# Polarisjame/DeepFake

Hardware: AMD Instinct MI355X
Metric: train clips/sec (32x224x224 video + 16kHz audio) at 1/2/4/8 MI355X (higher is better)
Workload: dtype bf16; 1 GPU; C2: Swin-T video 32x224x224 (window 8x7x7) + SwinV2 mel 224 + wav2vec2-base 4s@16kHz + FusionModel, full train step; global_batch=8, per_gpu_batch=8, parallelism=dp1, hip_graph=True, captured_overlap=False, captured_bn_broadcast=False, branch_streams=3, regularisers=True

## Files before the change

deepfake_amd/_lib.py:

```python
import ctypes as C
import os

import torch

_HERE = os.path.dirname(os.path.abspath(__file__))
LIB_PATH = os.environ.get("DFK_LIB") or os.path.join(_HERE, "libdfk.so")

F32, BF16 = 0, 1


class Drop(C.Structure):
    _fields_ = [("rng", C.c_void_p), ("mode", C.c_int32), ("site", C.c_int32), ("p", C.c_float),
                ("group_rows", C.c_int32), ("shared", C.c_int32)]


class View(C.Structure):
    _fields_ = [("ptr", C.c_void_p), ("ld", C.c_int64), ("bs0", C.c_int64), ("bs1", C.c_int64),
                ("conv_cg", C.c_int32), ("conv_stride", C.c_int32), ("conv_pad", C.c_int32),
                ("conv_rows", C.c_int32)]


class GemmArgs(C.Structure):
    _fields_ = [("a", View), ("b", View), ("c", C.c_void_p), ("bias", C.c_void_p), ("residual", C.c_void_p),
                ("aux", C.c_void_p), ("ldc", C.c_int64), ("cbs0", C.c_int64), ("cbs1", C.c_int64),
                ("ldr", C.c_int64), ("rbs0", C.c_int64), ("rbs1", C.c_int64), ("ldaux", C.c_int64),
                ("bias_bs1", C.c_int64),
                ("M", C.c_int32), ("N", C.c_int32), ("K", C.c_int32), ("dtype", C.c_int32),
                ("a_kmajor", C.c_int32), ("b_kmajor", C.c_int32), ("c_f32", C.c_int32), ("nz0", C.c_int32),
                ("nz1", C.c_int32), ("splitk", C.c_int32), ("act", C.c_int32), ("atomic", C.c_int32),
                ("beta", C.c_float), ("ws", C.c_void_p), ("rowsum", C.c_void_p), ("drop", Drop),
                ("alpha", C.c_float), ("mx_q", C.c_void_p), ("mx_s", C.c_void_p), ("mx_ldq", C.c_int64),
                ("mx_lds", C.c_int64)]


class MxOperand(C.Structure):
    _fields_ = [("q", C.c_void_p), ("s", C.c_void_p), ("ld", C.c_int64), ("lds", C.c_int64)]


class WattnArgs(C.Structure):
    _fields_ = [("q", C.c_void_p), ("k", C.c_void_p), ("v", C.c_void_p), ("out", C.c_void_p),
                ("rpb", C.c_void_p), ("pad_q", C.c_void_p), ("pad_k", C.c_void_p), ("pad_v", C.c_void_p),
                ("lse", C.c_void_p), ("mask", C.c_void_p), ("mask_nw", C.c_int64),
                ("ld_qkv", C.c_int64), ("ld_out", C.c_int64),
                ("B", C.c_int32), ("D", C.c_int32), ("H", C.c_int32), ("W", C.c_int32),
                ("wd", C.c_int32), ("wh", C.c_int32), ("ww", C.c_int32),
                ("fd", C.c_int32), ("fh", C.c_int32), ("fw", C.c_int32),
                ("sd", C.c_int32), ("sh", C.c_int32), ("sw", C.c_int32),
                ("heads", C.c_int32), ("hd", C.c_int32), ("dtype", C.c_int32), ("scale", C.c_float),
                ("tab", C.c_void_p), ("drop", Drop), ("klen", C.c_void_p)]
# ... 26 lines not shown
                ("Ho", C.c_int32), ("Wo", C.c_int32)]


class Im2colArgs(C.Structure):
    _fields_ = [("sb", C.c_int64), ("sc", C.c_int64), ("st", C.c_int64), ("sh", C.c_int64), ("sw", C.c_int64),
                ("B", C.c_int32), ("cin", C.c_int32), ("T", C.c_int32), ("H", C.c_int32), ("W", C.c_int32),
                ("pd", C.c_int32), ("ph", C.c_int32), ("pw", C.c_int32),
                ("Do", C.c_int32), ("Ho", C.c_int32), ("Wo", C.c_int32)]


_VP, _I64, _I32, _F = C.c_void_p, C.c_int64, C.c_int32, C.c_float
SIGNATURES = {
    "dfk_gemm": [C.POINTER(GemmArgs), _VP],
    "dfk_gemm_workspace": [C.POINTER(GemmArgs)],
    "dfk_gemm_dw_group": [C.POINTER(GemmArgs), _I32, _VP],
    "dfk_colsum": [_VP, C.c_int, _I64, _I64, _I64, _VP, _VP],
    "dfk_gemm_mx": [C.POINTER(GemmArgs), C.POINTER(MxOperand), C.POINTER(MxOperand), _VP],
    "dfk_mx_quant": [_VP, C.c_int, _I64, _I64, _I64, C.c_int, _VP, _I64, _VP, _VP],
    "dfk_layernorm_fwd": [_VP, _VP, _VP, _VP, _VP, _VP, _I64, _I32, _F, C.c_int, _VP, C.POINTER(Drop), _VP],
    "dfk_layernorm_bwd": [_VP, _VP, _VP, _VP, _VP, _VP, _VP, _VP, _I64, _I32, C.c_int, C.c_int, _VP,
                          C.POINTER(Drop), _VP, _VP],
    "dfk_layernorm_bwd_workspace": [_I64, _I32],
    "dfk_wattn_fwd": [C.POINTER(WattnArgs), _VP],
    "dfk_wattn_bwd": [C.POINTER(WattnBwdArgs), _VP],
    "dfk_wattn_bwd_workspace": [C.POINTER(WattnArgs)],
    "dfk_wattn_fwd_policy": [C.c_int32, C.c_int64],
    "dfk_wattn_bwd_policy": [C.c_int32, C.c_int32],
    "dfk_wattn_table_workspace": [C.POINTER(WattnArgs)],
    "dfk_wattn_table": [C.POINTER(WattnArgs), _VP],
    "dfk_patch_im2col": [_VP, C.c_int, _VP, C.c_int, C.POINTER(Im2colArgs), _VP],
# ... 147 lines not shown
```

deepfake_amd/csrc/gemm.hip:

```cpp
#include <mutex>

#include "common.h"

namespace {

constexpr int NT = 256;

struct SplitK {
  float* slab;
  uint32_t* cnt;
};

template <typename T> struct GT;
template <> struct GT<bf16raw> { static constexpr int BK = 64, VEC = 8, PADR = 8, PADK = 16; };
template <> struct GT<float> { static constexpr int BK = 32, VEC = 4, PADR = 4, PADK = 4; };

template <typename T, bool KMAJ, int ROWS>
struct Tile {
  static constexpr int TBK = GT<T>::BK;
  static constexpr int STRIDE = KMAJ ? ROWS + GT<T>::PADK : TBK + GT<T>::PADR;
  static constexpr int ELEMS = KMAJ ? TBK * STRIDE : ROWS * STRIDE;
};

template <bool CONV>
// ... 176 lines not shown
      if (full) { float c8v[8]; ld8<T>(C, c8v); for (int e = 0; e < 8; ++e) v[e] += g.beta * c8v[e]; }
      else for (int e = 0; e < 8; ++e) if (e < ncol) v[e] += g.beta * ldf<T>(C + e);
    }
    if (full) st8<T>(C, v);
    else for (int e = 0; e < 8; ++e) if (e < ncol) stf<T>(C + e, v[e]);
  }
}

template <typename T, int WT, bool MXO = false>
__device__ __forceinline__ void tile_epilogue(const dfk_gemm_args& g, float* smem, const f32x4 (&acc)[WT / 16][WT / 16],
                                              int lane, int wave, int wm, int wn, int bm, int bn, int z, int split,
                                              int tile, int evec, SplitK sk);
__device__ __forceinline__ int mx_scale_byte(float am);
__device__ __forceinline__ uint2 mx_pack8(const float (&v)[8], int e);

template <typename T, int WT, bool AK, bool BKM, bool VECOK, bool CONV, bool RS = false>
__global__ __launch_bounds__(256) void gemm_kernel(const dfk_gemm_args g, int kchunk, int evec, SplitK sk) {
  constexpr int BM = 2 * WT, BN = 2 * WT, MI = WT / 16;
  constexpr int VA = tile_vecs<T, BM>(), VB = tile_vecs<T, BN>();
  using TA = Tile<T, AK, BM>;
  using TB = Tile<T, BKM, BN>;
  constexpr int TBK = GT<T>::BK;
  constexpr int BUF = TA::ELEMS + TB::ELEMS;
  constexpr int ES = WT + 4;
  constexpr int SMEM_T = 2 * BUF > (4 * WT * ES * 4) / (int)sizeof(T) ? 2 * BUF : (4 * WT * ES * 4) / (int)sizeof(T);
  __shared__ __attribute__((aligned(16))) T smem[SMEM_T];
  const int tid = threadIdx.x, lane = tid & 63, wave = tid >> 6;
  const int wm = wave >> 1, wn = wave & 1;
  int tn, tmi;
  {
    const int nwg = gridDim.x * gridDim.y, bid = blockIdx.y * gridDim.x + blockIdx.x;
    const int xcd = bid & 7, q = nwg >> 3, rr = nwg & 7;
    const int nid = (xcd < rr ? xcd * (q + 1) : rr * (q + 1) + (xcd - rr) * q) + (bid >> 3);
    tn = nid % gridDim.x;
    tmi = nid / gridDim.x;
  }
  const int bn = tn * BN, bm = tmi * BM;
  int z = blockIdx.z;
  const int split = z % g.splitk;
  z /= g.splitk;
  const int z0 = z / g.nz1, z1 = z % g.nz1;
  const T* A = reinterpret_cast<const T*>(g.a.ptr) + z0 * g.a.bs0 + z1 * g.a.bs1;
  const T* B = reinterpret_cast<const T*>(g.b.ptr) + z0 * g.b.bs0 + z1 * g.b.bs1;
  const int kbeg = split * kchunk;
  const int kend = min(g.K, kbeg + kchunk);

  f32x4 acc[MI][MI];
#pragma unroll
  for (int i = 0; i < MI; ++i)
#pragma unroll
    for (int j = 0; j < MI; ++j) acc[i][j] = f32x4{0.f, 0.f, 0.f, 0.f};
  const bool do_rs = RS && tn == 0 && wn == 0;
  f32x4 accr[MI];
// ... 73 lines not shown
      load_tile<T, BKM, BN, VECOK, CONV>(B, g.b, bn, g.N, kn, kend, tid, rb[nx]);
    }
  }

  if (RS && do_rs && (lane & 15) == 0) {
#pragma unroll
    for (int mi = 0; mi < MI; ++mi)
#pragma unroll
      for (int r = 0; r < 4; ++r) {
        const int row = bm + wm * WT + mi * 16 + (lane >> 4) * 4 + r;
        if (row < g.M) atomicAdd(g.rowsum + row, accr[mi][r]);
      }
  }
  __syncthreads();
  tile_epilogue<T, WT>(g, reinterpret_cast<float*>(smem), acc, lane, wave, wm, wn, bm, bn, z, split,
                       (z * (int)gridDim.y + tmi) * (int)gridDim.x + tn, evec, sk);
}

template <typename T, int WT, bool MXO>
__device__ __forceinline__ void tile_epilogue(const dfk_gemm_args& g, float* smem, const f32x4 (&acc)[WT / 16][WT / 16],
                                              int lane, int wave, int wm, int wn, int bm, int bn, int z, int split,
                                              int tile, int evec, SplitK sk) {
  constexpr int MI = WT / 16, ES = WT + 4;
  const int z0 = z / g.nz1, z1 = z % g.nz1;
  float* es = smem + wave * WT * ES;
#pragma unroll
  for (int mi = 0; mi < MI; ++mi)
#pragma unroll
    for (int ni = 0; ni < MI; ++ni)
#pragma unroll
      for (int r = 0; r < 4; ++r) es[(mi * 16 + (lane >> 4) * 4 + r) * ES + ni * 16 + (lane & 15)] = acc[mi][ni][r];
// ... 165 lines not shown
    const bf16raw* hi = img + (k + 4) * ROWS + ((c ^ kmaj_swz<ROWS>(k + 4)) << 3) + (p & 1) * 4;
    const short4v a = __builtin_amdgcn_ds_read_tr16_b64_v4i16((lds_short4*)(lo));
    const short4v b = __builtin_amdgcn_ds_read_tr16_b64_v4i16((lds_short4*)(hi));
    short8 u = {a[0], a[1], a[2], a[3], b[0], b[1], b[2], b[3]};
    return __builtin_bit_cast(bf16x8, u);
  }
}

__host__ __device__ __forceinline__ long view_extent(const dfk_view& v, long rows, long cols) {
  if (v.conv_cg > 0) return ((long)(v.conv_rows - 1) * v.ld + v.conv_cg) * 2;
  return ((rows - 1) * v.ld + cols) * 2;
}

constexpr int kRsPartialMin = 32;

template <int WT, int NWM, int NWN, bool AK, bool BKM, bool RS, bool CONV>
__device__ __forceinline__ void gemm_dma_body(const dfk_gemm_args& g, int kchunk, int evec, SplitK sk, const dim3 bid,
                                              const dim3 grid) {
  constexpr int NWV = NWM * NWN, BM = NWM * WT, BN = NWN * WT, MI = WT / 16, BK = 64, S = kStages;
  constexpr int STAGE = (BM + BN) * BK;
  constexpr int ES = WT + 4;
  constexpr int SMEM = S * STAGE * 2 > NWV * WT * ES * 4 ? S * STAGE * 2 : NWV * WT * ES * 4;
  __shared__ __attribute__((aligned(16))) float smem_f[SMEM / 4];
  bf16raw* smem = reinterpret_cast<bf16raw*>(smem_f);
  const int tid = threadIdx.x, lane = tid & 63;
  const int wave = __builtin_amdgcn_readfirstlane(tid >> 6);
  const int wm = wave / NWN, wn = wave % NWN;
  int tn, tmi, z;
  const int nwg = grid.x * grid.y;
  if (g.atomic && g.splitk % 8 == 0 && (int)grid.z == g.splitk && nwg > 1) {
    const int lin = bid.z * nwg + bid.y * grid.x + bid.x;
    const int j = lin >> 3, i = j % nwg;
    z = (j / nwg) * 8 + (lin & 7);
    tn = i % grid.x;
    tmi = i / grid.x;
  } else {
    const int b2 = bid.y * grid.x + bid.x;
    const int xcd = b2 & 7, q = nwg >> 3, rr = nwg & 7;
    const int nid = (xcd < rr ? xcd * (q + 1) : rr * (q + 1) + (xcd - rr) * q) + (b2 >> 3);
    tn = nid % grid.x;
    tmi = nid / grid.x;
    z = bid.z;
  }
  const int bn = tn * BN, bm = tmi * BM;
  const int split = z % g.splitk;
  z /= g.splitk;
  const int z0 = z / g.nz1, z1 = z % g.nz1;
  const bf16raw* A = reinterpret_cast<const bf16raw*>(g.a.ptr) + z0 * g.a.bs0 + z1 * g.a.bs1;
  const bf16raw* B = reinterpret_cast<const bf16raw*>(g.b.ptr) + z0 * g.b.bs0 + z1 * g.b.bs1;
  const __amdgpu_buffer_rsrc_t ra = __builtin_amdgcn_make_buffer_rsrc(
      const_cast<bf16raw*>(A), (short)0, (int)(AK ? view_extent(g.a, g.K, g.M) : view_extent(g.a, g.M, g.K)), 0x00020000);
  const __amdgpu_buffer_rsrc_t rb = __builtin_amdgcn_make_buffer_rsrc(
      const_cast<bf16raw*>(B), (short)0, (int)(BKM ? view_extent(g.b, g.K, g.N) : view_extent(g.b, g.N, g.K)), 0x00020000);
  const int kbeg = split * kchunk;
  const int kend = min(g.K, kbeg + kchunk);
  const int ntile = kend > kbeg ? (kend - kbeg + BK - 1) / BK : 0;

  auto issue = [&](int kt, bf16raw* st) {
    Dma<AK, BM, NWV, CONV>::issue(ra, g.a, bm, g.M, kt, kend, st, wave, lane);
// ... 69 lines not shown
            else atomicAdd(g.rowsum + row, accr[h][r]);
          }
        }
    }
  }
  asm volatile("s_waitcnt vmcnt(0) lgkmcnt(0)" ::: "memory");
  __syncthreads();
  tile_epilogue<bf16raw, WT>(g, smem_f, acc, lane, wave, wm, wn, bm, bn, z, split,
                             (z * (int)grid.y + tmi) * (int)grid.x + tn, evec, sk);
}

template <int WT, int NWM, int NWN, bool AK, bool BKM, bool RS, bool CONV>
__global__ __launch_bounds__(NWM * NWN * 64) void gemm_dma_kernel(const dfk_gemm_args g, int kchunk, int evec,
                                                                  SplitK sk) {
  gemm_dma_body<WT, NWM, NWN, AK, BKM, RS, CONV>(g, kchunk, evec, sk, blockIdx, gridDim);
}

constexpr int kDwGroupMax = 8;
struct DwProblem {
  const void *a, *b;
  float *c, *rowsum;
  int32_t M, N, K;
  int32_t lda, ldb, ldc;
  int32_t splitk, kchunk;
  int32_t gx, gy;
};
struct DwGroup {
  DwProblem p[kDwGroupMax];
  int32_t prefix[kDwGroupMax + 1];
  int32_t n;
// ... 508 lines not shown
    if (hipMemsetAsync(p, 0, kTickets * 4, s) != hipSuccess || hipStreamSynchronize(s) != hipSuccess) {
      (void)hipFree(p);
      return nullptr;
    }
    arena[dev] = static_cast<uint32_t*>(p);
  }
  if (cursor[dev] + n > kTickets) cursor[dev] = 0;
  uint32_t* t = arena[dev] + cursor[dev];
  cursor[dev] += (n + 63) & ~63L;
  return t;
}

extern "C" int dfk_gemm(const dfk_gemm_args* g, hipStream_t s) {
  if (!g || g->mx_q) return DFK_EINVAL;
  return g->dtype == DFK_BF16 ? launch<bf16raw>(*g, s) : launch<float>(*g, s);
}

bool dw_group_plan(const dfk_gemm_args& g, DwProblem& r, int& wt) {
  if (g.dtype != DFK_BF16 || !g.a_kmajor || !g.b_kmajor || !g.c_f32 || g.mx_q) return false;
  if (!g.a.ptr || !g.b.ptr || !g.c || g.M <= 0 || g.N <= 0 || g.K <= 0) return false;
  if (g.nz0 != 1 || g.nz1 != 1 || g.a.conv_cg > 0 || g.b.conv_cg > 0) return false;
  if (g.bias || g.residual || g.aux || g.act || g.drop.mode || (g.alpha != 0.f && g.alpha != 1.f)) return false;
  if (g.splitk < 1 || (g.atomic != 0) != (g.splitk > 1) || (!g.atomic && g.beta != 1.f)) return false;
  if (g.rowsum && g.splitk >= kRsPartialMin) return false;
  if (g.K >= 16384) return false;
  if (!dma_vec(g)) return false;
  if (g.a.ld > 0x7fffffffL || g.b.ld > 0x7fffffffL || g.ldc > 0x7fffffffL) return false;
  if (auto_splitk(g) != 1) return false;
  wt = pick_tile(g).wt;
  const long gx = dfk_cdiv(g.N, 2 * wt), gy = dfk_cdiv(g.M, 2 * wt);
// ... 162 lines not shown
```

deepfake_amd/csrc/misc.hip:

```cpp
#include <math.h>

#include "common.h"

namespace {

template <typename TI, typename TO>
__global__ void im2col_kernel(const TI* __restrict__ x, TO* __restrict__ out, dfk_im2col_args a, long total) {
  const long idx = (long)blockIdx.x * blockDim.x + threadIdx.x;
  if (idx >= total) return;
  const int K = a.cin * a.pd * a.ph * a.pw;
  const long row = idx / K;
  const int k = (int)(idx - row * K);
  const int kw = k % a.pw, kh = (k / a.pw) % a.ph, kd = (k / (a.pw * a.ph)) % a.pd, c = k / (a.pw * a.ph * a.pd);
  const int w = (int)(row % a.Wo), h = (int)((row / a.Wo) % a.Ho), d = (int)((row / ((long)a.Wo * a.Ho)) % a.Do);
  const long b = row / ((long)a.Wo * a.Ho * a.Do);
  const int t = d * a.pd + kd, y = h * a.ph + kh, xx = w * a.pw + kw;
  float v = 0.f;
  if (t < a.T && y < a.H && xx < a.W) v = ldf<TI>(x + b * a.sb + c * a.sc + t * a.st + (long)y * a.sh + (long)xx * a.sw);
  stf<TO>(out + idx, v);
}

template <typename TO>
__global__ __launch_bounds__(256) void im2col_rows_kernel(const float* __restrict__ x, TO* __restrict__ out,
                                                          dfk_im2col_args a) {
// ... 489 lines not shown
__global__ __launch_bounds__(256) void wn_apply_bwd_kernel(const float* __restrict__ v, const float* __restrict__ g,
                                                           const float* __restrict__ norm, const float* __restrict__ s,
                                                           const float* __restrict__ dw2, int Cg, int k,
                                                           float* __restrict__ dv) {
  extern __shared__ float wsm[];
  const int o = blockIdx.x, n = Cg * k;
  for (int p = threadIdx.x; p < n; p += blockDim.x) wsm[p] = dw2[(long)o * n + p];
  __syncthreads();
  for (int p = threadIdx.x; p < n; p += blockDim.x) {
    const int i = p / k, kk = p % k;
    const float nk = norm[kk], gk = g[kk];
    dv[(long)o * n + p] += gk / nk * wsm[kk * Cg + i] - gk * s[kk] / (nk * nk * nk) * v[(long)o * n + p];
  }
}

}

extern "C" int dfk_posconv_wnorm_fwd(const float* v, const float* g, int32_t C, int32_t Cg, int32_t k, float* norm,
                                     float* ws, void* w2, void* w3, int dtype, hipStream_t s) {
  if (!v || !g || !norm || !ws || !w2 || !w3 || C <= 0 || Cg <= 0 || k <= 0 || C % Cg) return DFK_EINVAL;
  if (dtype != DFK_BF16 && dtype != DFK_F32) return DFK_EINVAL;
  const size_t lds = sizeof(float) * (size_t)Cg * k;
  if (lds > 64 * 1024) return DFK_EINVAL;
  hipLaunchKernelGGL(wn_partial_kernel, dim3(C), dim3(256), 0, s, v, nullptr, Cg, k, ws);
  hipLaunchKernelGGL(wn_reduce_kernel, dim3(k), dim3(256), 0, s, ws, C, k, norm, nullptr);
  if (dtype == DFK_BF16)
    hipLaunchKernelGGL(wn_apply_fwd_kernel<bf16raw>, dim3(C, 2), dim3(256), lds, s, v, g, norm, Cg, k, (bf16raw*)w2,
                       (bf16raw*)w3);
  else
    hipLaunchKernelGGL(wn_apply_fwd_kernel<float>, dim3(C, 2), dim3(256), lds, s, v, g, norm, Cg, k, (float*)w2,
// ... 17 lines not shown
```

deepfake_amd/functional.py:

```python
import torch

from . import kernels as K


def _orig(p):
    if p is None or hasattr(p, "_dfk_store") or not isinstance(p, torch.Tensor):
        return p
    from .params import PARAM_BY_PTR
    q = PARAM_BY_PTR.get(p.data_ptr())
    return q if q is not None and q.shape == p.shape else p


def compute_weight(p, dtype):
    if p is None:
        return None
    p = _orig(p)
    if p.dtype == dtype:
        return p
    sh = getattr(p, "_dfk_shadow", None)
    if sh is not None and sh.dtype == dtype:
        return sh
    return p.detach().to(dtype)


# ... 445 lines not shown
        for i, p in enumerate((weight, gamma, beta)):
            grad_use(ctx, 1 + i, p)
        ctx.save_for_backward(wave, w, weight, gamma, beta, stats)
        ctx.eps = eps
        return out

    @staticmethod
    def backward(ctx, dout):
        wave, w, weight, gamma, beta, stats = ctx.saved_tensors
        dw, dg, db = grad_sink(weight), grad_sink(gamma), grad_sink(beta)
        K.w2v_conv0_bwd(wave.float().contiguous(), w, gamma.detach().float(), beta.detach().float(), ctx.eps, stats,
                        dout.contiguous(), dw.view(512, 10), dg, db)
        return None, grad_done(weight, dw), grad_done(gamma, dg), grad_done(beta, db), None, None


def _conv1d_gemm_fwd(x, weight, stride, out, bias=None, act=0, aux=None):
    B, Tin, Cin = x.shape
    Cout, _, k = weight.shape
    Tout = out.shape[1]
    w2 = weight.detach().permute(0, 2, 1).reshape(Cout, k * Cin).to(x.dtype).contiguous()
    K.gemm(x, Cin, False, w2, k * Cin, False, Tout, Cout, k * Cin, out, Cout, dtype=K.L.dt(x),
           bias=compute_weight(bias, x.dtype), act=act, aux=aux, ldaux=Cout if aux is not None else 0, nz=(B, 1),
           a_bs=(Tin * Cin, 0), c_bs=(Tout * Cout, 0), a_conv=(Cin, stride, 0, Tin))
    return w2


def _conv1d_gemm_bwd(x, w2, dpre, stride, k, need_dx):
    B, Tin, Cin = x.shape
    Tout, Cout = dpre.shape[1:]
    dt = K.L.dt(x)
    dw2 = torch.zeros(Cout, k * Cin, device=x.device)
    tiles = -(-Cout // 128) * -(-(k * Cin) // 128)
    K.gemm(dpre, Cout, True, x, Cin, True, Cout, k * Cin, Tout, dw2, k * Cin, dtype=dt, c_f32=True, atomic=True,
           splitk=max(1, min(K.splitk_for(tiles * B, Tout, 128), 16)), nz=(B, 1), a_bs=(Tout * Cout, 0),
           b_bs=(Tin * Cin, 0), b_conv=(Cin, stride, 0, Tin))
    dx = None
    if need_dx:
        dx = torch.zeros(B, Tin, Cin, device=x.device, dtype=x.dtype)
        for kk in range(k):
            K.gemm(dpre, Cout, False, w2[:, kk * Cin:], k * Cin, True, Tout, Cin, Cout, dx[:, kk:], stride * Cin,
                   dtype=dt, beta=1.0, nz=(B, 1), a_bs=(Tout * Cout, 0), c_bs=(Tin * Cin, 0))
    return dx, dw2.view(Cout, k, Cin).permute(0, 2, 1)


class ConvGeluFn(torch.autograd.Function):

    @staticmethod
    def forward(ctx, x, weight, stride):
        B, Tin, _ = x.shape
        Cout, _, k = weight.shape
        y = torch.empty(B, (Tin - k) // stride + 1, Cout, device=x.device, dtype=x.dtype)
        pre = torch.empty_like(y)
        w2 = _conv1d_gemm_fwd(x, weight, stride, y, act=1, aux=pre)
        ctx.save_for_backward(x, w2, pre)
        ctx.meta = (stride, k)
        return y

    @staticmethod
    def backward(ctx, dy):
        x, w2, pre = ctx.saved_tensors
        stride, k = ctx.meta
        dx, dw = _conv1d_gemm_bwd(x, w2, K.gelu_bwd(dy.contiguous(), pre), stride, k, ctx.needs_input_grad[0])
        return dx, dw, None


class W2VConv0LNFn(torch.autograd.Function):

    @staticmethod
    def forward(ctx, wave, weight, bias, gamma, beta, eps, dtype):
        w = weight.detach().float().reshape(512, 10).contiguous()
        f32 = lambda p: None if p is None else p.detach().float()
        out, stats = K.w2v_conv0_ln_fwd(wave.float().contiguous(), w, f32(bias), f32(gamma), f32(beta), eps, dtype)
        for i, p in enumerate((weight, bias, gamma, beta)):
            if p is not None:
                grad_use(ctx, 1 + i, p)
        ctx.save_for_backward(wave, w, weight, bias, gamma, beta, stats)
        return out

# ... 3 lines not shown
        f32 = lambda p: None if p is None else p.detach().float()
        dw, dg, dbe = grad_sink(weight), grad_sink(gamma), grad_sink(beta)
        db = grad_sink(bias) if bias is not None else None
        K.w2v_conv0_ln_bwd(wave.float().contiguous(), w, f32(bias), f32(gamma), f32(beta), stats, dout.contiguous(),
                           dw.view(512, 10), db, dg, dbe)
        return (None, grad_done(weight, dw), grad_done(bias, db) if bias is not None else None, grad_done(gamma, dg),
                grad_done(beta, dbe), None, None)


class ConvLNGeluFn(torch.autograd.Function):

    @staticmethod
    def forward(ctx, x, weight, bias, gamma, beta, stride, eps):
        B, Tin, _ = x.shape
        Cout, _, k = weight.shape
        pre = torch.empty(B, (Tin - k) // stride + 1, Cout, device=x.device, dtype=x.dtype)
        w2 = _conv1d_gemm_fwd(x, weight, stride, pre, bias=bias)
        y, stats = K.w2v_ln_gelu_fwd(pre, gamma.detach().float(), beta.detach().float(), eps)
        for i, p in ((2, bias), (3, gamma), (4, beta)):
            if p is not None:
                grad_use(ctx, i, p)
        ctx.save_for_backward(x, w2, pre, stats, bias, gamma, beta)
        ctx.meta = (stride, k)
        return y

    @staticmethod
    def backward(ctx, dy):
        x, w2, pre, stats, bias, gamma, beta = ctx.saved_tensors
        stride, k = ctx.meta
        dg, dbe = grad_sink(gamma), grad_sink(beta)
        db = grad_sink(bias) if bias is not None else None
        dpre = K.w2v_ln_gelu_bwd(dy.contiguous(), pre, gamma.detach().float(), beta.detach().float(), stats, dg, dbe, db)
        dx, dw = _conv1d_gemm_bwd(x, w2, dpre, stride, k, ctx.needs_input_grad[0])
        return (dx, dw, grad_done(bias, db) if bias is not None else None, grad_done(gamma, dg), grad_done(beta, dbe),
                None, None)


def _posconv_gemm_fwd(x, w2, bias, groups, k):
    B, T, C = x.shape
    Cg = C // groups
    dt = x.dtype
    y = torch.empty_like(x)
    pre = torch.empty_like(x)
    K.gemm(x, C, False, w2, k * Cg, False, T, Cg, k * Cg, y, C, dtype=K.L.dt(x), bias=compute_weight(bias, dt),
           bias_bs1=Cg, act=1, aux=pre, ldaux=C, residual=x, ldr=C, nz=(B, groups), a_bs=(T * C, Cg),
           b_bs=(0, Cg * k * Cg), c_bs=(T * C, Cg), r_bs=(T * C, Cg), a_conv=(Cg, 1, k // 2, T))
    return y, pre

# ... 372 lines not shown
```

deepfake_amd/kernels.py:

```python
import ctypes
import math

import torch

from . import _lib as L

_CU_TARGET_BLOCKS = 256


def _view(t, ld, bs0=0, bs1=0, conv=None):
    v = L.View()
    v.ptr = t.data_ptr()
    v.ld, v.bs0, v.bs1 = int(ld), int(bs0), int(bs1)
    if conv:
        v.conv_cg, v.conv_stride, v.conv_pad, v.conv_rows = (int(c) for c in conv)
    return v


def gemm(a, a_ld, a_kmajor, b, b_ld, b_kmajor, M, N, K, c, ldc, **kw):
    _gemm_launch(_gemm_args(a, a_ld, a_kmajor, b, b_ld, b_kmajor, M, N, K, c, ldc, **kw), c)


def _gemm_args(a, a_ld, a_kmajor, b, b_ld, b_kmajor, M, N, K, c, ldc, *, dtype, c_f32=False, bias=None,
               residual=None, ldr=0, aux=None, ldaux=0, act=0, beta=0.0, atomic=False, splitk=1,
# ... 546 lines not shown
    scratch = torch.empty(max(L.lib().dfk_w2v_ln_gelu_bwd_workspace(rows) // 4, 4), device=x.device,
                          dtype=torch.float32)
    L.check(L.lib().dfk_w2v_ln_gelu_bwd(L.ptr(dy), L.ptr(x), rows, C, L.ptr(gamma), L.ptr(beta), L.ptr(stats),
                                        L.ptr(dx), L.dt(x), L.ptr(scratch), scratch.numel() * 4, L.ptr(dgamma),
                                        L.ptr(dbeta), L.ptr(dbias), L.stream()), "w2v_ln_gelu_bwd")
    return dx


def gelu_bwd(dy, pre, out=None):
    if out is None:
        out = torch.empty_like(dy)
    L.check(L.lib().dfk_gelu_bwd(L.ptr(dy), L.ptr(pre), L.ptr(out), dy.numel(), L.dt(dy), L.stream()), "gelu_bwd")
    return out


def posconv_wnorm_fwd(v, g, C, Cg, k, norm, ws, w2, w3):
    L.check(L.lib().dfk_posconv_wnorm_fwd(L.ptr(v), L.ptr(g), C, Cg, k, L.ptr(norm), L.ptr(ws), L.ptr(w2), L.ptr(w3),
                                          L.dt(w2), L.stream()), "posconv_wnorm_fwd")


def posconv_wnorm_bwd(v, g, norm, dw2, C, Cg, k, ws, dv, dg):
    L.check(L.lib().dfk_posconv_wnorm_bwd(L.ptr(v), L.ptr(g), L.ptr(norm), L.ptr(dw2), C, Cg, k, L.ptr(ws), L.ptr(dv),
                                          L.ptr(dg), L.stream()), "posconv_wnorm_bwd")


def cast(x, dtype):
    y = torch.empty(x.shape, device=x.device, dtype=dtype)
    L.check(L.lib().dfk_cast(L.ptr(x), L.dt(x), L.ptr(y), L.dt(y), x.numel(), L.stream()), "cast")
    return y

# ... 321 lines not shown
```

deepfake_amd/models/wav2vec2.py:

```python
import json

import torch
import torch.nn as nn
from torch.nn.utils import parametrizations

from .. import functional as Fn
from .. import kernels as K
from .. import rng


class Wav2Vec2Config:

    def __init__(self, **kw):
        self.conv_dim = kw.get("conv_dim", [512] * 7)
        self.conv_kernel = kw.get("conv_kernel", [10, 3, 3, 3, 3, 2, 2])
        self.conv_stride = kw.get("conv_stride", [5, 2, 2, 2, 2, 2, 2])
        self.conv_bias = kw.get("conv_bias", False)
        self.feat_extract_norm = kw.get("feat_extract_norm", "group")
        self.hidden_size = kw.get("hidden_size", 768)
        self.num_attention_heads = kw.get("num_attention_heads", 12)
        self.intermediate_size = kw.get("intermediate_size", 3072)
        self.num_hidden_layers = kw.get("num_hidden_layers", 12)
        self.num_conv_pos_embeddings = kw.get("num_conv_pos_embeddings", 128)
        self.num_conv_pos_embedding_groups = kw.get("num_conv_pos_embedding_groups", 16)
# ... 74 lines not shown
                           "group" if i == 0 else None)
                for i in range(len(config.conv_dim))])
        self.compute_dtype = torch.float32

    def forward(self, input_values):
        l0 = self.conv_layers[0]
        if self.layer_norm_path:
            x = Fn.W2VConv0LNFn.apply(input_values, l0.conv.weight, l0.conv.bias, l0.layer_norm.weight,
                                      l0.layer_norm.bias, l0.layer_norm.eps, self.compute_dtype)
            for layer in self.conv_layers[1:]:
                x = Fn.ConvLNGeluFn.apply(x, layer.conv.weight, layer.conv.bias, layer.layer_norm.weight,
                                          layer.layer_norm.bias, layer.stride, layer.layer_norm.eps)
            return x
        x = Fn.W2VConv0Fn.apply(input_values, l0.conv.weight, l0.layer_norm.weight, l0.layer_norm.bias,
                                l0.layer_norm.eps, self.compute_dtype)
        for layer in self.conv_layers[1:]:
            x = Fn.ConvGeluFn.apply(x, layer.conv.weight, layer.stride)
        return x


class Wav2Vec2FeatureProjection(nn.Module):

    def __init__(self, config):
        super().__init__()
        self.layer_norm = nn.LayerNorm(config.conv_dim[-1], eps=config.layer_norm_eps)
        self.projection = nn.Linear(config.conv_dim[-1], config.hidden_size)
        self.dropout = rng.Drop(config.feat_proj_dropout)

    def forward(self, x):
        n = Fn.layer_norm(x, self.layer_norm)
        d = self.dropout.spec() if self.dropout.active(self.training) else None
        return Fn.linear(n, self.projection.weight, self.projection.bias, drop=d), n

# ... 219 lines not shown
```

include/dfk.h:

```cpp
#ifndef DFK_H
#define DFK_H
#include <stdint.h>
#include <hip/hip_runtime.h>

#ifdef __cplusplus
extern "C" {
#endif

#define DFK_F32 0
#define DFK_BF16 1
#define DFK_EINVAL (-1)
#define DFK_ENOTSUP (-2)

typedef struct {
  const int64_t* rng;
  int32_t mode;
  int32_t site;
  float p;
  int32_t group_rows;
  int32_t shared;
} dfk_drop;

typedef struct {
  const void* ptr;
// ... 26 lines not shown
  int32_t act;
  int32_t atomic;
  float beta;
  void* ws;
  float* rowsum;
  dfk_drop drop;
  float alpha;
  uint8_t* mx_q;
  uint32_t* mx_s;
  int64_t mx_ldq, mx_lds;
} dfk_gemm_args;
int dfk_gemm(const dfk_gemm_args* g, hipStream_t stream);
int64_t dfk_gemm_workspace(const dfk_gemm_args* g);
int dfk_gemm_dw_group(const dfk_gemm_args* problems, int32_t n, hipStream_t stream);

typedef struct {
  const uint8_t* q;
  const uint32_t* s;
  int64_t ld;
  int64_t lds;
} dfk_mx_operand;
int dfk_mx_quant(const void* x, int dtype, int64_t rows, int64_t cols, int64_t ldx, int transpose, uint8_t* q,
                 int64_t ldq, uint32_t* s, hipStream_t stream);
int dfk_gemm_mx(const dfk_gemm_args* g, const dfk_mx_operand* a, const dfk_mx_operand* b, hipStream_t stream);

int dfk_colsum(const void* x, int dtype, int64_t rows, int64_t cols, int64_t ld, float* out, hipStream_t stream);

int dfk_layernorm_fwd(const void* x, const void* w, const void* b, void* y, float* mean, float* rstd,
                      int64_t rows, int32_t C, float eps, int dtype, const void* residual, const dfk_drop* drop,
                      hipStream_t stream);
// ... 260 lines not shown
```

Measured before the change: 296.5 clips/s.

## Compute wav2vec2 conv dx via stride-phase decomposition in one kernel

Replaces the per-tap loop of dx GEMMs (k launches with beta=1 accumulation over a zeroed buffer) with a stride-phase decomposition: each output phase becomes an implicit-conv GEMM over reordered weights, and all phases run in a single launch. A new pack kernel builds both the forward weight layout and the flipped dx weight layout in one launch for all stacked conv layers. The conv layers 1..n are fused into one autograd function, so gelu backward is folded into the dx GEMM epilogue (act=2 with aux), the zero fill of dx is dropped, and dw is skipped when it is not needed. This cuts launches and read-modify-write traffic in the wav2vec2 feature extractor, at the cost of extra kernel variants and a packed weight buffer per step.

```diff
diff --git a/deepfake_amd/_lib.py b/deepfake_amd/_lib.py
--- a/deepfake_amd/_lib.py
+++ b/deepfake_amd/_lib.py
@@ -33,6 +33,16 @@
                 ("mx_lds", C.c_int64)]
 
 
+class ConvPhase(C.Structure):
+    _fields_ = [("b_off", C.c_int64), ("c_off", C.c_int64), ("M", C.c_int32), ("K", C.c_int32),
+                ("conv_pad", C.c_int32), ("reserved", C.c_int32)]
+
+
+class ConvPackLayer(C.Structure):
+    _fields_ = [("w", C.c_void_p), ("wf", C.c_void_p), ("wdx", C.c_void_p), ("Cout", C.c_int32), ("Cin", C.c_int32),
+                ("k", C.c_int32), ("stride", C.c_int32)]
+
+
 class MxOperand(C.Structure):
     _fields_ = [("q", C.c_void_p), ("s", C.c_void_p), ("ld", C.c_int64), ("lds", C.c_int64)]
 
@@ -89,6 +99,8 @@
     "dfk_gemm": [C.POINTER(GemmArgs), _VP],
     "dfk_gemm_workspace": [C.POINTER(GemmArgs)],
     "dfk_gemm_dw_group": [C.POINTER(GemmArgs), _I32, _VP],
+    "dfk_gemm_conv_phases": [C.POINTER(GemmArgs), C.POINTER(ConvPhase), _I32, _VP],
+    "dfk_conv1d_pack": [C.POINTER(ConvPackLayer), _I32, C.c_int, C.c_int, _VP],
     "dfk_colsum": [_VP, C.c_int, _I64, _I64, _I64, _VP, _VP],
     "dfk_gemm_mx": [C.POINTER(GemmArgs), C.POINTER(MxOperand), C.POINTER(MxOperand), _VP],
     "dfk_mx_quant": [_VP, C.c_int, _I64, _I64, _I64, C.c_int, _VP, _I64, _VP, _VP],
diff --git a/deepfake_amd/csrc/gemm.hip b/deepfake_amd/csrc/gemm.hip
--- a/deepfake_amd/csrc/gemm.hip
+++ b/deepfake_amd/csrc/gemm.hip
@@ -214,8 +214,9 @@
 __device__ __forceinline__ int mx_scale_byte(float am);
 __device__ __forceinline__ uint2 mx_pack8(const float (&v)[8], int e);
 
-template <typename T, int WT, bool AK, bool BKM, bool VECOK, bool CONV, bool RS = false>
-__global__ __launch_bounds__(256) void gemm_kernel(const dfk_gemm_args g, int kchunk, int evec, SplitK sk) {
+template <typename T, int WT, bool AK, bool BKM, bool VECOK, bool CONV, bool RS, bool PH>
+__device__ __forceinline__ void gemm_body(const dfk_gemm_args& g, int kchunk, int evec, SplitK sk, const dim3 bid,
+                                          const dim3 grid) {
   constexpr int BM = 2 * WT, BN = 2 * WT, MI = WT / 16;
   constexpr int VA = tile_vecs<T, BM>(), VB = tile_vecs<T, BN>();
   using TA = Tile<T, AK, BM>;
@@ -229,14 +230,15 @@
   const int wm = wave >> 1, wn = wave & 1;
   int tn, tmi;
   {
-    const int nwg = gridDim.x * gridDim.y, bid = blockIdx.y * gridDim.x + blockIdx.x;
-    const int xcd = bid & 7, q = nwg >> 3, rr = nwg & 7;
-    const int nid = (xcd < rr ? xcd * (q + 1) : rr * (q + 1) + (xcd - rr) * q) + (bid >> 3);
-    tn = nid % gridDim.x;
-    tmi = nid / gridDim.x;
+    const int nwg = grid.x * grid.y, b2 = bid.y * grid.x + bid.x;
+    const int xcd = b2 & 7, q = nwg >> 3, rr = nwg & 7;
+    const int nid = (xcd < rr ? xcd * (q + 1) : rr * (q + 1) + (xcd - rr) * q) + (b2 >> 3);
+    tn = nid % grid.x;
+    tmi = nid / grid.x;
   }
   const int bn = tn * BN, bm = tmi * BM;
-  int z = blockIdx.z;
+  if (PH && bm >= g.M) return;
+  int z = bid.z;
   const int split = z % g.splitk;
   z /= g.splitk;
   const int z0 = z / g.nz1, z1 = z % g.nz1;
@@ -340,7 +342,12 @@
   }
   __syncthreads();
   tile_epilogue<T, WT>(g, reinterpret_cast<float*>(smem), acc, lane, wave, wm, wn, bm, bn, z, split,
-                       (z * (int)gridDim.y + tmi) * (int)gridDim.x + tn, evec, sk);
+                       (z * (int)grid.y + tmi) * (int)grid.x + tn, evec, sk);
+}
+
+template <typename T, int WT, bool AK, bool BKM, bool VECOK, bool CONV, bool RS = false>
+__global__ __launch_bounds__(256) void gemm_kernel(const dfk_gemm_args g, int kchunk, int evec, SplitK sk) {
+  gemm_body<T, WT, AK, BKM, VECOK, CONV, RS, false>(g, kchunk, evec, sk, blockIdx, gridDim);
 }
 
 template <typename T, int WT, bool MXO>
@@ -536,7 +543,7 @@
 
 constexpr int kRsPartialMin = 32;
 
-template <int WT, int NWM, int NWN, bool AK, bool BKM, bool RS, bool CONV>
+template <int WT, int NWM, int NWN, bool AK, bool BKM, bool RS, bool CONV, bool PH = false>
 __device__ __forceinline__ void gemm_dma_body(const dfk_gemm_args& g, int kchunk, int evec, SplitK sk, const dim3 bid,
                                               const dim3 grid) {
   constexpr int NWV = NWM * NWN, BM = NWM * WT, BN = NWN * WT, MI = WT / 16, BK = 64, S = kStages;
@@ -565,6 +572,7 @@
     z = bid.z;
   }
   const int bn = tn * BN, bm = tmi * BM;
+  if (PH && bm >= g.M) return;
   const int split = z % g.splitk;
   z /= g.splitk;
   const int z0 = z / g.nz1, z1 = z % g.nz1;
@@ -664,6 +672,45 @@
 __global__ __launch_bounds__(NWM * NWN * 64) void gemm_dma_kernel(const dfk_gemm_args g, int kchunk, int evec,
                                                                   SplitK sk) {
   gemm_dma_body<WT, NWM, NWN, AK, BKM, RS, CONV>(g, kchunk, evec, sk, blockIdx, gridDim);
+}
+
+struct ConvPhases {
+  dfk_conv_phase p[DFK_CONV_PHASES_MAX];
+};
+
+template <typename T>
+__device__ __forceinline__ int conv_phase_args(const dfk_gemm_args& g0, const ConvPhases& P, dfk_gemm_args& g) {
+  const int nb = g0.nz0 * g0.nz1;
+  const int pi = __builtin_amdgcn_readfirstlane((int)blockIdx.z / nb);
+  const dfk_conv_phase& ph = P.p[pi];
+  g = g0;
+  g.M = ph.M;
+  g.K = ph.K;
+  g.a.conv_pad = ph.conv_pad;
+  g.b.ptr = reinterpret_cast<const T*>(g0.b.ptr) + ph.b_off;
+  g.c = reinterpret_cast<T*>(g0.c) + ph.c_off;
+  if (g0.aux) g.aux = reinterpret_cast<T*>(g0.aux) + ph.c_off;
+  if (g0.residual) g.residual = reinterpret_cast<const T*>(g0.residual) + ph.c_off;
+  return (int)blockIdx.z - pi * nb;
+}
+
+template <int WT>
+__global__ __launch_bounds__(256) void gemm_dma_phase_kernel(const dfk_gemm_args g0, const ConvPhases P, int evec) {
+  dfk_gemm_args g;
+  const int z = conv_phase_args<bf16raw>(g0, P, g);
+  gemm_dma_body<WT, 2, 2, false, true, false, true, true>(g, (g.K + 63) / 64 * 64, evec, SplitK{nullptr, nullptr},
+                                                          dim3(blockIdx.x, blockIdx.y, z),
+                                                          dim3(gridDim.x, gridDim.y, g0.nz0 * g0.nz1));
+}
+
+template <typename T, int WT, bool VECOK>
+__global__ __launch_bounds__(256) void gemm_phase_kernel(const dfk_gemm_args g0, const ConvPhases P, int evec) {
+  dfk_gemm_args g;
+  const int z = conv_phase_args<T>(g0, P, g);
+  constexpr int TBK = GT<T>::BK;
+  gemm_body<T, WT, false, true, VECOK, true, false, true>(g, (g.K + TBK - 1) / TBK * TBK, evec,
+                                                          SplitK{nullptr, nullptr}, dim3(blockIdx.x, blockIdx.y, z),
+                                                          dim3(gridDim.x, gridDim.y, g0.nz0 * g0.nz1));
 }
 
 constexpr int kDwGroupMax = 8;
@@ -1202,6 +1249,65 @@
 extern "C" int dfk_gemm(const dfk_gemm_args* g, hipStream_t s) {
   if (!g || g->mx_q) return DFK_EINVAL;
   return g->dtype == DFK_BF16 ? launch<bf16raw>(*g, s) : launch<float>(*g, s);
+}
+
+template <typename T>
+static int launch_conv_phases(const dfk_gemm_args& g, const dfk_conv_phase* ph, int n, hipStream_t s) {
+  constexpr int VEC = GT<T>::VEC;
+  ConvPhases P = {};
+  bool dma = true, vec = true, evec = true;
+  int maxM = 0;
+  for (int i = 0; i < n; ++i) {
+    const dfk_conv_phase& p = ph[i];
+    if (p.M < 0 || p.K < 0 || p.conv_pad < 0 || p.b_off < 0 || p.c_off < 0 || p.K % g.a.conv_cg) return DFK_EINVAL;
+    P.p[i] = p;
+    dfk_gemm_args q = g;
+    q.M = p.M;
+    q.K = p.K;
+    q.a.conv_pad = p.conv_pad;
+    q.b.ptr = reinterpret_cast<const T*>(g.b.ptr) + p.b_off;
+    q.c = reinterpret_cast<T*>(g.c) + p.c_off;
+    if (g.aux) q.aux = reinterpret_cast<T*>(g.aux) + p.c_off;
+    if (g.residual) q.residual = reinterpret_cast<const T*>(g.residual) + p.c_off;
+    dma = dma && dma_vec(q);
+    vec = vec && views_vec(q, VEC);
+    evec = evec && epi_vec(q);
+    maxM = std::max(maxM, p.M);
+  }
+  if (maxM == 0 || g.N <= 0) return 0;
+  dfk_gemm_args gm = g;
+  gm.M = maxM;
+  gm.K = ph[0].K;
+  gm.nz0 = g.nz0 * n;
+  const int wt = pick_wt(gm);
+  const dim3 grid(dfk_cdiv(g.N, 2 * wt), dfk_cdiv(maxM, 2 * wt), g.nz0 * g.nz1 * n);
+  if (grid.y > 65535 || grid.z > 65535) return DFK_EINVAL;
+  const int ev = evec ? 1 : 0;
+  void (*k)(const dfk_gemm_args, const ConvPhases, int);
+  if constexpr (sizeof(T) == 2) {
+    if (dma) k = wt == 64 ? gemm_dma_phase_kernel<64> : gemm_dma_phase_kernel<32>;
+    else if (vec) k = wt == 64 ? gemm_phase_kernel<T, 64, true> : gemm_phase_kernel<T, 32, true>;
+    else k = wt == 64 ? gemm_phase_kernel<T, 64, false> : gemm_phase_kernel<T, 32, false>;
+  } else {
+    if (vec) k = wt == 64 ? gemm_phase_kernel<T, 64, true> : gemm_phase_kernel<T, 32, true>;
+    else k = wt == 64 ? gemm_phase_kernel<T, 64, false> : gemm_phase_kernel<T, 32, false>;
+  }
+  hipLaunchKernelGGL(k, grid, dim3(256), 0, s, g, P, ev);
+  DFK_CHECK_LAUNCH();
+  return 0;
+}
+
+extern "C" int dfk_gemm_conv_phases(const dfk_gemm_args* gp, const dfk_conv_phase* phases, int32_t n, hipStream_t s) {
+  if (!gp || !phases || n < 1 || n > DFK_CONV_PHASES_MAX) return DFK_EINVAL;
+  const dfk_gemm_args& g = *gp;
+  if (!g.a.ptr || !g.b.ptr || !g.c || g.mx_q) return DFK_EINVAL;
+  if (g.dtype != DFK_BF16 && g.dtype != DFK_F32) return DFK_EINVAL;
+  if (g.a.conv_cg <= 0 || g.a.conv_stride != 1 || g.a.conv_rows <= 0 || g.a_kmajor) return DFK_EINVAL;
+  if (g.b.conv_cg > 0 || !g.b_kmajor) return DFK_EINVAL;
+  if (g.splitk != 1 || g.atomic || g.c_f32 || g.rowsum || g.drop.mode || g.nz0 < 1 || g.nz1 < 1)
+    return DFK_EINVAL;
+  if ((g.act != 0 && g.act != 2) || (g.act == 2 && !g.aux)) return DFK_EINVAL;
+  return g.dtype == DFK_BF16 ? launch_conv_phases<bf16raw>(g, phases, n, s) : launch_conv_phases<float>(g, phases, n, s);
 }
 
 bool dw_group_plan(const dfk_gemm_args& g, DwProblem& r, int& wt) {
diff --git a/deepfake_amd/csrc/misc.hip b/deepfake_amd/csrc/misc.hip
--- a/deepfake_amd/csrc/misc.hip
+++ b/deepfake_amd/csrc/misc.hip
@@ -527,6 +527,70 @@
   }
 }
 
+struct ConvPack {
+  dfk_conv_pack_layer l[DFK_CONV_PACK_MAX];
+  int32_t prefix[DFK_CONV_PACK_MAX + 1];
+  int32_t n;
+};
+
+template <typename S, typename D>
+__global__ __launch_bounds__(256) void conv_pack_kernel(const ConvPack P) {
+  extern __shared__ float csm[];
+  const int b = blockIdx.x;
+  int li = 0;
+#pragma unroll
+  for (int i = 1; i < DFK_CONV_PACK_MAX; ++i) li += (i < P.n && b >= P.prefix[i]) ? 1 : 0;
+  li = __builtin_amdgcn_readfirstlane(li);
+  const dfk_conv_pack_layer& L = P.l[li];
+  const int co = b - P.prefix[li], Cin = L.Cin, Cout = L.Cout, k = L.k, s = L.stride, n = Cin * k;
+  const S* src = reinterpret_cast<const S*>(L.w) + (long)co * n;
+  for (int p = threadIdx.x; p < n; p += blockDim.x) csm[p] = ldf<S>(src + p);
+  __syncthreads();
+  D* wf = reinterpret_cast<D*>(L.wf) + (long)co * n;
+  D* wdx = reinterpret_cast<D*>(L.wdx);
+  for (int p = threadIdx.x; p < n; p += blockDim.x) {
+    const int kk = p / Cin, ci = p - kk * Cin;
+    const float v = csm[ci * k + kk];
+    stf<D>(wf + p, v);
+    if (wdx) {
+      const int ph = kk % s, j = kk / s;
+      int blk = (k - ph + s - 1) / s - 1 - j;
+      for (int q = 0; q < ph; ++q) blk += (k - q + s - 1) / s;
+      stf<D>(wdx + ((long)blk * Cout + co) * Cin + ci, v);
+    }
+  }
+}
+
+}
+
+extern "C" int dfk_conv1d_pack(const dfk_conv_pack_layer* layers, int32_t n, int src_dtype, int dst_dtype,
+                               hipStream_t s) {
+  if (!layers || n < 1 || n > DFK_CONV_PACK_MAX) return DFK_EINVAL;
+  if ((src_dtype != DFK_BF16 && src_dtype != DFK_F32) || (dst_dtype != DFK_BF16 && dst_dtype != DFK_F32))
+    return DFK_EINVAL;
+  ConvPack P = {};
+  size_t lds = 0;
+  for (int i = 0; i < n; ++i) {
+    const dfk_conv_pack_layer& l = layers[i];
+    if (!l.w || !l.wf || l.Cout <= 0 || l.Cin <= 0 || l.k <= 0 || l.stride <= 0) return DFK_EINVAL;
+    P.l[i] = l;
+    P.prefix[i + 1] = P.prefix[i] + l.Cout;
+    const size_t need = sizeof(float) * (size_t)l.Cin * l.k;
+    lds = need > lds ? need : lds;
+  }
+  P.n = n;
+  if (lds > 64 * 1024) return DFK_EINVAL;
+  const dim3 grid((unsigned)P.prefix[n]), blk(256);
+  if (src_dtype == DFK_F32 && dst_dtype == DFK_BF16)
+    hipLaunchKernelGGL((conv_pack_kernel<float, bf16raw>), grid, blk, lds, s, P);
+  else if (src_dtype == DFK_F32)
+    hipLaunchKernelGGL((conv_pack_kernel<float, float>), grid, blk, lds, s, P);
+  else if (dst_dtype == DFK_BF16)
+    hipLaunchKernelGGL((conv_pack_kernel<bf16raw, bf16raw>), grid, blk, lds, s, P);
+  else
+    hipLaunchKernelGGL((conv_pack_kernel<bf16raw, float>), grid, blk, lds, s, P);
+  DFK_CHECK_LAUNCH();
+  return 0;
 }
 
 extern "C" int dfk_posconv_wnorm_fwd(const float* v, const float* g, int32_t C, int32_t Cg, int32_t k, float* norm,
diff --git a/deepfake_amd/functional.py b/deepfake_amd/functional.py
--- a/deepfake_amd/functional.py
+++ b/deepfake_amd/functional.py
@@ -483,33 +483,32 @@
         return None, grad_done(weight, dw), grad_done(gamma, dg), grad_done(beta, db), None, None
 
 
-def _conv1d_gemm_fwd(x, weight, stride, out, bias=None, act=0, aux=None):
+def _conv_pack(weights, strides, dtype):
+    return K.conv1d_pack([w.detach().contiguous() for w in weights], strides, dtype)
+
+
+def _conv1d_gemm_fwd(x, wf, k, stride, out, bias=None, act=0, aux=None):
     B, Tin, Cin = x.shape
-    Cout, _, k = weight.shape
+    Cout = wf.shape[0]
     Tout = out.shape[1]
-    w2 = weight.detach().permute(0, 2, 1).reshape(Cout, k * Cin).to(x.dtype).contiguous()
-    K.gemm(x, Cin, False, w2, k * Cin, False, Tout, Cout, k * Cin, out, Cout, dtype=K.L.dt(x),
+    K.gemm(x, Cin, False, wf, k * Cin, False, Tout, Cout, k * Cin, out, Cout, dtype=K.L.dt(x),
            bias=compute_weight(bias, x.dtype), act=act, aux=aux, ldaux=Cout if aux is not None else 0, nz=(B, 1),
            a_bs=(Tin * Cin, 0), c_bs=(Tout * Cout, 0), a_conv=(Cin, stride, 0, Tin))
-    return w2
-
-
-def _conv1d_gemm_bwd(x, w2, dpre, stride, k, need_dx):
+
+
+def _conv1d_gemm_bwd(x, wdx, dpre, stride, k, need_dw, need_dx, aux=None):
     B, Tin, Cin = x.shape
     Tout, Cout = dpre.shape[1:]
-    dt = K.L.dt(x)
-    dw2 = torch.zeros(Cout, k * Cin, device=x.device)
-    tiles = -(-Cout // 128) * -(-(k * Cin) // 128)
-    K.gemm(dpre, Cout, True, x, Cin, True, Cout, k * Cin, Tout, dw2, k * Cin, dtype=dt, c_f32=True, atomic=True,
-           splitk=max(1, min(K.splitk_for(tiles * B, Tout, 128), 16)), nz=(B, 1), a_bs=(Tout * Cout, 0),
-           b_bs=(Tin * Cin, 0), b_conv=(Cin, stride, 0, Tin))
-    dx = None
-    if need_dx:
-        dx = torch.zeros(B, Tin, Cin, device=x.device, dtype=x.dtype)
-        for kk in range(k):
-            K.gemm(dpre, Cout, False, w2[:, kk * Cin:], k * Cin, True, Tout, Cin, Cout, dx[:, kk:], stride * Cin,
-                   dtype=dt, beta=1.0, nz=(B, 1), a_bs=(Tout * Cout, 0), c_bs=(Tin * Cin, 0))
-    return dx, dw2.view(Cout, k, Cin).permute(0, 2, 1)
+    dw = None
+    if need_dw:
+        dw2 = torch.zeros(Cout, k * Cin, device=x.device)
+        tiles = -(-Cout // 128) * -(-(k * Cin) // 128)
+        K.gemm(dpre, Cout, True, x, Cin, True, Cout, k * Cin, Tout, dw2, k * Cin, dtype=K.L.dt(x), c_f32=True,
+               atomic=True, splitk=max(1, min(K.splitk_for(tiles * B, Tout, 128), 16)), nz=(B, 1),
+               a_bs=(Tout * Cout, 0), b_bs=(Tin * Cin, 0), b_conv=(Cin, stride, 0, Tin))
+        dw = dw2.view(Cout, k, Cin).permute(0, 2, 1)
+    dx = K.conv1d_dx(dpre, wdx, k, stride, Tin, aux=aux) if need_dx else None
+    return dx, dw
 
 
 class ConvGeluFn(torch.autograd.Function):
@@ -518,19 +517,55 @@
     def forward(ctx, x, weight, stride):
         B, Tin, _ = x.shape
         Cout, _, k = weight.shape
+        x = x.contiguous()
         y = torch.empty(B, (Tin - k) // stride + 1, Cout, device=x.device, dtype=x.dtype)
         pre = torch.empty_like(y)
-        w2 = _conv1d_gemm_fwd(x, weight, stride, y, act=1, aux=pre)
-        ctx.save_for_backward(x, w2, pre)
+        (wf, wdx), = _conv_pack([weight], [stride], x.dtype)
+        _conv1d_gemm_fwd(x, wf, k, stride, y, act=1, aux=pre)
+        ctx.save_for_backward(x, wdx, pre)
         ctx.meta = (stride, k)
         return y
 
     @staticmethod
     def backward(ctx, dy):
-        x, w2, pre = ctx.saved_tensors
+        x, wdx, pre = ctx.saved_tensors
         stride, k = ctx.meta
-        dx, dw = _conv1d_gemm_bwd(x, w2, K.gelu_bwd(dy.contiguous(), pre), stride, k, ctx.needs_input_grad[0])
+        dx, dw = _conv1d_gemm_bwd(x, wdx, K.gelu_bwd(dy.contiguous(), pre), stride, k, ctx.needs_input_grad[1],
+                                  ctx.needs_input_grad[0])
         return dx, dw, None
+
+
+class ConvStackFn(torch.autograd.Function):
+
+    @staticmethod
+    def forward(ctx, x, strides, *weights):
+        ops = _conv_pack(weights, strides, x.dtype)
+        x = x.contiguous()
+        xs, pres = [], []
+        for (wf, _), w, s in zip(ops, weights, strides):
+            B, Tin, _ = x.shape
+            Cout, _, k = w.shape
+            y = torch.empty(B, (Tin - k) // s + 1, Cout, device=x.device, dtype=x.dtype)
+            pre = torch.empty_like(y)
+            _conv1d_gemm_fwd(x, wf, k, s, y, act=1, aux=pre)
+            xs.append(x)
+            pres.append(pre)
+            x = y
+        ctx.save_for_backward(*xs, *pres, *[o[1] for o in ops])
+        ctx.strides, ctx.taps = tuple(strides), tuple(w.shape[2] for w in weights)
+        return x
+
+    @staticmethod
+    def backward(ctx, dy):
+        n, sv = len(ctx.taps), ctx.saved_tensors
+        xs, pres, wdxs = sv[:n], sv[n:2 * n], sv[2 * n:]
+        dpre = K.gelu_bwd(dy.contiguous(), pres[-1])
+        dws = [None] * n
+        for i in reversed(range(n)):
+            dpre, dws[i] = _conv1d_gemm_bwd(xs[i], wdxs[i], dpre, ctx.strides[i], ctx.taps[i],
+                                            ctx.needs_input_grad[2 + i], i > 0 or ctx.needs_input_grad[0],
+                                            aux=pres[i - 1] if i > 0 else None)
+        return (dpre, None, *dws)
 
 
 class W2VConv0LNFn(torch.autograd.Function):
@@ -564,24 +599,26 @@
     def forward(ctx, x, weight, bias, gamma, beta, stride, eps):
         B, Tin, _ = x.shape
         Cout, _, k = weight.shape
+        x = x.contiguous()
         pre = torch.empty(B, (Tin - k) // stride + 1, Cout, device=x.device, dtype=x.dtype)
-        w2 = _conv1d_gemm_fwd(x, weight, stride, pre, bias=bias)
+        (wf, wdx), = _conv_pack([weight], [stride], x.dtype)
+        _conv1d_gemm_fwd(x, wf, k, stride, pre, bias=bias)
         y, stats = K.w2v_ln_gelu_fwd(pre, gamma.detach().float(), beta.detach().float(), eps)
         for i, p in ((2, bias), (3, gamma), (4, beta)):
             if p is not None:
                 grad_use(ctx, i, p)
-        ctx.save_for_backward(x, w2, pre, stats, bias, gamma, beta)
+        ctx.save_for_backward(x, wdx, pre, stats, bias, gamma, beta)
         ctx.meta = (stride, k)
         return y
 
     @staticmethod
     def backward(ctx, dy):
-        x, w2, pre, stats, bias, gamma, beta = ctx.saved_tensors
+        x, wdx, pre, stats, bias, gamma, beta = ctx.saved_tensors
         stride, k = ctx.meta
         dg, dbe = grad_sink(gamma), grad_sink(beta)
         db = grad_sink(bias) if bias is not None else None
         dpre = K.w2v_ln_gelu_bwd(dy.contiguous(), pre, gamma.detach().float(), beta.detach().float(), stats, dg, dbe, db)
-        dx, dw = _conv1d_gemm_bwd(x, w2, dpre, stride, k, ctx.needs_input_grad[0])
+        dx, dw = _conv1d_gemm_bwd(x, wdx, dpre, stride, k, ctx.needs_input_grad[1], ctx.needs_input_grad[0])
         return (dx, dw, grad_done(bias, db) if bias is not None else None, grad_done(gamma, dg), grad_done(beta, dbe),
                 None, None)
 
diff --git a/deepfake_amd/kernels.py b/deepfake_amd/kernels.py
--- a/deepfake_amd/kernels.py
+++ b/deepfake_amd/kernels.py
@@ -584,6 +584,55 @@
     return out
 
 
+def conv1d_phase_plan(k, s, Tin):
+    if k < 1 or s < 1 or Tin < k:
+        raise ValueError(f"conv1d_phase_plan: k={k} s={s} Tin={Tin}")
+    plan, blk = [], 0
+    for p in range(s):
+        J = max(0, -(-(k - p) // s))
+        U = max(0, -(-(Tin - p) // s))
+        plan.append({"p": p, "J": J, "U": U, "pad": max(J - 1, 0), "blk": blk,
+                     "taps": [p + s * (J - 1 - j) for j in range(J)]})
+        blk += J
+    return plan
+
+
+def conv1d_pack(weights, strides, dtype, dx=True):
+    n = len(weights)
+    arr = (L.ConvPackLayer * n)()
+    out = []
+    for i, (w, s) in enumerate(zip(weights, strides)):
+        Cout, Cin, k = w.shape
+        if not w.is_contiguous() or w.dtype != weights[0].dtype:
+            raise ValueError("conv1d_pack: contiguous weights of one dtype expected")
+        wf = torch.empty(Cout, k * Cin, device=w.device, dtype=dtype)
+        wdx = torch.empty(k * Cout, Cin, device=w.device, dtype=dtype) if dx else None
+        a = arr[i]
+        a.w, a.wf, a.wdx = w.data_ptr(), wf.data_ptr(), wdx.data_ptr() if dx else None
+        a.Cout, a.Cin, a.k, a.stride = Cout, Cin, k, int(s)
+        L.ptr(w)
+        out.append((wf, wdx))
+    L.check(L.lib().dfk_conv1d_pack(arr, n, L.dt(weights[0]), L.dt(out[0][0]), L.stream()), "conv1d_pack")
+    return out
+
+
+def conv1d_dx(dpre, wdx, k, stride, Tin, aux=None):
+    B, Tout, Cout = dpre.shape
+    Cin = wdx.shape[1]
+    dx = torch.empty(B, Tin, Cin, device=dpre.device, dtype=dpre.dtype)
+    plan = conv1d_phase_plan(k, stride, Tin)
+    g = _gemm_args(dpre, Cout, False, wdx, Cin, True, 0, Cin, 0, dx, stride * Cin, dtype=L.dt(dpre),
+                   act=2 if aux is not None else 0, aux=aux, ldaux=stride * Cin if aux is not None else 0,
+                   nz=(B, 1), a_bs=(Tout * Cout, 0), c_bs=(Tin * Cin, 0), a_conv=(Cout, 1, 0, Tout))
+    ph = (L.ConvPhase * len(plan))()
+    for q, e in zip(ph, plan):
+        q.M, q.K, q.conv_pad = e["U"], e["J"] * Cout, e["pad"]
+        q.b_off = e["blk"] * Cout * Cin if e["J"] else 0
+        q.c_off = e["p"] * Cin
+    L.check(L.lib().dfk_gemm_conv_phases(g, ph, len(plan), L.stream()), f"conv1d_dx k={k} s={stride} Tin={Tin}")
+    return dx
+
+
 def posconv_wnorm_fwd(v, g, C, Cg, k, norm, ws, w2, w3):
     L.check(L.lib().dfk_posconv_wnorm_fwd(L.ptr(v), L.ptr(g), C, Cg, k, L.ptr(norm), L.ptr(ws), L.ptr(w2), L.ptr(w3),
                                           L.dt(w2), L.stream()), "posconv_wnorm_fwd")
diff --git a/deepfake_amd/models/wav2vec2.py b/deepfake_amd/models/wav2vec2.py
--- a/deepfake_amd/models/wav2vec2.py
+++ b/deepfake_amd/models/wav2vec2.py
@@ -112,9 +112,10 @@
             return x
         x = Fn.W2VConv0Fn.apply(input_values, l0.conv.weight, l0.layer_norm.weight, l0.layer_norm.bias,
                                 l0.layer_norm.eps, self.compute_dtype)
-        for layer in self.conv_layers[1:]:
-            x = Fn.ConvGeluFn.apply(x, layer.conv.weight, layer.stride)
-        return x
+        rest = self.conv_layers[1:]
+        if len(rest) == 0:
+            return x
+        return Fn.ConvStackFn.apply(x, tuple(layer.stride for layer in rest), *[layer.conv.weight for layer in rest])
 
 
 class Wav2Vec2FeatureProjection(nn.Module):
diff --git a/include/dfk.h b/include/dfk.h
--- a/include/dfk.h
+++ b/include/dfk.h
@@ -64,6 +64,25 @@
 int64_t dfk_gemm_workspace(const dfk_gemm_args* g);
 int dfk_gemm_dw_group(const dfk_gemm_args* problems, int32_t n, hipStream_t stream);
 
+#define DFK_CONV_PHASES_MAX 8
+typedef struct {
+  int64_t b_off;
+  int64_t c_off;
+  int32_t M, K;
+  int32_t conv_pad;
+  int32_t reserved;
+} dfk_conv_phase;
+int dfk_gemm_conv_phases(const dfk_gemm_args* g, const dfk_conv_phase* phases, int32_t n, hipStream_t stream);
+
+#define DFK_CONV_PACK_MAX 8
+typedef struct {
+  const void* w;
+  void* wf;
+  void* wdx;
+  int32_t Cout, Cin, k, stride;
+} dfk_conv_pack_layer;
+int dfk_conv1d_pack(const dfk_conv_pack_layer* layers, int32_t n, int src_dtype, int dst_dtype, hipStream_t stream);
+
 typedef struct {
   const uint8_t* q;
   const uint32_t* s;
```

New measurement: 296.8 clips/s (median of 3 runs). About the same (+0.1%).
